# FerrisMind/candle-video

Measured on AMD Instinct MI355X. Metric: frames/sec end-to-end LTX-Video-2B 512x768x97; DiT step ms; VAE decode ms, higher is better.
Workload: dtype bf16; 1 GPU; LTX-Video-0.9.8-2B-distilled 512x768x97, 7 steps (configs.rs:223-240), untiled VAE decode; preset=0.9.8-2b-distilled, denoise_steps=7, parallelism=replicas x1 (no data-path collective)

## Files before the change

### candle-video_amd/csrc/capi_ops.hip

```cpp
#include "model_util.h"
#include "../../include/ltxhip_ops.h"

static inline int dtc(int d) { return d == 1 ? LTX_DT_BF16 : LTX_DT_F32; }

extern "C" int ltx_op_linear(const void* x, const void* w, const void* bias, void* y, int M, int N, int K, int dtype, int epi,
                             const void* resid, const float* gate, int rows_per_batch, ltx_stream stream) {
    if (!x || !w || !y) LTX_FAIL(LTX_ERR_ARG, "ltx_op_linear: null tensor");
    if (epi < 0 || epi > 3) LTX_FAIL(LTX_ERR_ARG, "ltx_op_linear: epi must be 0..3");
    if ((epi == 2 || epi == 3) && !resid) LTX_FAIL(LTX_ERR_ARG, "ltx_op_linear: residual epilogue needs resid");
    if (epi == 2 && (!gate || rows_per_batch < 1)) LTX_FAIL(LTX_ERR_ARG, "ltx_op_linear: gated epilogue needs gate");
    GemmArgs g; g.A = x; g.W = w; g.C = y; g.bias = bias; g.resid = resid; g.gate = gate;
    g.M = M; g.N = N; g.K = K; g.lda = K; g.ldc = N; g.ldr = N; g.rows_per_batch = rows_per_batch > 0 ? rows_per_batch : 1; g.gate_stride = N;
    return ltx_launch_gemm(g, dtc(dtype), epi, (hipStream_t)stream);
}

extern "C" int64_t ltx_op_ring_packed_bytes(int N, int K) { return (int64_t)ltx_ring_packed_bytes(N, K); }
extern "C" int ltx_op_ring_pack(const void* w, int N, int K, void* out, ltx_stream stream) { return ltx_pack_ring_weights(w, N, K, out, (hipStream_t)stream); }
extern "C" int ltx_op_linear_packed(const void* x, const void* w, const void* w_packed, const void* bias, void* y, int M, int N, int K, int epi,
                                    const void* resid, const float* gate, int rows_per_batch, ltx_stream stream) {
    if (!x || !w || !w_packed || !y) LTX_FAIL(LTX_ERR_ARG, "ltx_op_linear_packed: null tensor");
    if (epi < 0 || epi > 3) LTX_FAIL(LTX_ERR_ARG, "ltx_op_linear_packed: epi must be 0..3");
    if ((epi == 2 || epi == 3) && !resid) LTX_FAIL(LTX_ERR_ARG, "ltx_op_linear_packed: residual epilogue needs resid");
    if (epi == 2 && (!gate || rows_per_batch < 1)) LTX_FAIL(LTX_ERR_ARG, "ltx_op_linear_packed: gated epilogue needs gate");
    GemmArgs g; g.A = x; g.W = w; g.Wp = w_packed; g.C = y; g.bias = bias; g.resid = resid; g.gate = gate;
// ... 135 lines not shown
    if (hipMemcpy(dtab, tab, sizeof(tab), hipMemcpyHostToDevice) != hipSuccess) rc = LTX_ERR_HIP;
    if (rc == LTX_OK) {
        TimeVec tv; tv.n = n;
        for (int i = 0; i < n; ++i) tv.t[i] = timesteps_host[i];
        rc = ltx_launch_sinusoid(out, dtc(dtype), tv, dtab, 128, dtc(dtype) == LTX_DT_BF16, multiplier, (hipStream_t)stream);
        if (rc == LTX_OK && hipStreamSynchronize((hipStream_t)stream) != hipSuccess) rc = LTX_ERR_HIP;
    }
    (void)hipFree(dtab);
    return rc;
}

extern "C" int ltx_op_qknorm_rope(void* x, int64_t rows, int D, int ld, const void* weight, float eps,
                                  const float* cos, const float* sin, int dtype, ltx_stream stream) {
    if (!x || !weight) LTX_FAIL(LTX_ERR_ARG, "ltx_op_qknorm_rope: null tensor");
    QkNormRopeArgs a; a.x = x; a.rows = rows; a.D = D; a.ld = ld; a.nseg = 1; a.w0 = weight; a.eps = eps; a.cos = cos; a.sin = sin;
    return ltx_launch_qknorm_rope(a, dtc(dtype), (hipStream_t)stream);
}

extern "C" int ltx_op_rope_table(float* cos, float* sin, const float* coords, int B, int F, int H, int W, int D,
                                 const float* rope_scale_host, ltx_stream stream) {
    if (!cos || !sin) LTX_FAIL(LTX_ERR_ARG, "ltx_op_rope_table: null tensor");
    int steps = D / 6; if (steps < 1) steps = 1;
    std::vector<float> fr(steps);
    const float theta_ln = (float)std::log(10000.0);
    for (int i = 0; i < steps; ++i) {
        float lin = steps <= 1 ? 0.0f : (float)i * (float)(1.0 / (double)(steps - 1));
        fr[i] = (float)std::exp((double)(lin * theta_ln)) * (float)(M_PI / 2.0);
    }
    float* dfr = nullptr;
    HIP_TRY(hipMalloc((void**)&dfr, sizeof(float) * steps));
// ... 166 lines not shown
```

### candle-video_amd/csrc/dit.hip

```cpp
#include <cstring>
#include <deque>
#include "model_util.h"
#include "options.h"
#include "../../include/ltxhip_cond.h"
#include "lora.h"

struct DitBlock {
    LinearW qkv1, o1, q2, kv2, o2, ff1, ff2;
    void *nq1 = nullptr, *nk1 = nullptr, *nq2 = nullptr, *nk2 = nullptr;
};

struct DitCtx {
    const void* enc = nullptr; const float* mask = nullptr;
    int B = 0, K = 0, iodt = 0; bool valid = false;
    bool fold_q2 = false;
    DevBuf kv, bias;
    bool compact = false;
    DevBuf kvc, biasc, kidx, kcount;
    void release() { kv.release(); bias.release(); kvc.release(); biasc.release(); kidx.release(); kcount.release(); valid = false; }
};

struct DitTimeEntry {
    float t[8] = {0}; int B = 0; hipStream_t stream = nullptr; bool valid = false; uint64_t used = 0;
    DevBuf ada, adaf;
// ... 18 lines not shown
    int device = 0;
    int D = 0;
    LinearW proj_in, te1, te2, te_lin, cap1, cap2, proj_out;
    void* sst_final = nullptr;
    void* sst_blocks = nullptr;
    std::vector<DitBlock> blocks;
    float* rope_freqs = nullptr;
    float* inv_freq = nullptr;
    std::vector<int> skip_blocks;
    std::deque<DitCtx> ctxs;
    bool ctx_mode = false;
    std::deque<DitTimeEntry> tcache; uint64_t tclock = 0;
    std::deque<DitWfold> wcache;
    std::deque<DitGroupEntry> gcache;
    bool wfold_off = false;
    struct { bool valid = false; const float* coords = nullptr; float rs[3] = {0, 0, 0}; bool has_rs = false; int B = 0, S = 0, F = 0, H = 0, W = 0; hipStream_t stream = nullptr; } rope_key;
    void invalidate_weight_derived() {
        for (auto& e : wcache) e.valid = false;
        for (auto& e : ctxs) e.valid = false;
        for (auto& e : tcache) e.cfold_valid = false;
        for (auto& e : gcache) e.cfold_valid = false;
    }
    void release_scaled_weights() { for (auto& e : wcache) e.release(); }
    void release_caches() { auto all = [](auto& c) { for (auto& e : c) e.release(); c.clear(); }; all(ctxs); all(tcache); all(wcache); all(gcache); }
    std::vector<void*> owned;
    struct LoraSlots { void* base[7] = {nullptr}; void* merged[7] = {nullptr}; };
    std::vector<LoraSlots> lora_w;
    int n_adapters = 0;
    DevBuf xin, encin, h, n, qkv, attn, ff, c1, encp, kv2, tproj, e1, emb, embs, temb, ada, adaf, cosb, sinb, bias, orig, orig_hsq, outT, rsq, hsq, parts;
    void free_all() {
        for (void* p : owned) if (p) (void)hipFree(p);
        owned.clear();
        for (auto& ls : lora_w) for (void*& p : ls.merged) if (p) { (void)hipFree(p); p = nullptr; }
        lora_w.clear();
        DevBuf* bs[] = {&xin, &encin, &h, &n, &qkv, &attn, &ff, &c1, &encp, &kv2, &tproj, &e1, &emb, &embs, &temb, &ada, &adaf, &cosb, &sinb, &bias, &orig, &orig_hsq, &outT, &rsq, &hsq, &parts};
        for (DevBuf* b : bs) b->release();
        release_caches();
    }
};

namespace {

int own_linear(ltx_dit* m, const WeightMap& wm, const std::string& prefix, int in, int out, LinearW* l) {
    LTX_TRY(ltx_load_linear(wm, prefix, in, out, m->dtype, l));
    m->owned.push_back(l->w); if (l->b) m->owned.push_back(l->b);
    return LTX_OK;
}
int own_tensor(ltx_dit* m, const WeightMap& wm, const std::string& name, int64_t numel, void** out) {
    LTX_TRY(ltx_load_tensor(wm, name, numel, m->dtype, out));
    m->owned.push_back(*out);
// ... 370 lines not shown
    RopeTableArgs r;
    r.cos = m->cosb.as<float>(); r.sin = m->sinb.as<float>(); r.freqs = m->rope_freqs;
    r.B = p.B; r.D = p.D;
    if (video_coords) {
        r.use_coords = 1; r.coords = video_coords; r.F = 1; r.H = 1; r.W = p.S;
        r.gscale[0] = (float)(1.0 / 20.0); r.gscale[1] = (float)(1.0 / 2048.0); r.gscale[2] = (float)(1.0 / 2048.0);
    } else {
        r.F = num_frames; r.H = height; r.W = width;
        if (rope_scale) {
            r.gscale[0] = (float)((double)rope_scale[0] * c.patch_size_t / 20.0);
            r.gscale[1] = (float)((double)rope_scale[1] * c.patch_size / 2048.0);
            r.gscale[2] = (float)((double)rope_scale[2] * c.patch_size / 2048.0);
        }
    }
    LTX_TRY(ltx_launch_rope_table(r, s));
    rk.coords = video_coords; rk.B = p.B; rk.S = p.S; rk.F = num_frames; rk.H = height; rk.W = width; rk.stream = s;
    rk.has_rs = rope_scale != nullptr; if (rope_scale) memcpy(rk.rs, rope_scale, sizeof(rk.rs));
    rk.valid = m->ctx_mode;
    return LTX_OK;
}

struct DitCarry {
    bool hsq_valid = false;
    bool hs_valid = false;
    bool hsq_saved = false;
    bool pending = false; const float* pend_gate = nullptr; const void* pend_bias = nullptr;
    void take_pending(RowNormArgs& rn, const ltx_dit* m, const DitPlan& p) {
        if (!pending) return;
        rn.parts = m->parts.as<float>(); rn.nparts = p.ff2_parts; rn.part_stride = p.M * p.D; rn.d_bias = pend_bias; rn.d_gate = pend_gate; rn.d_gate_stride = 6 * p.D;
        rn.x_out = m->h.p; pending = false;
// ... 31 lines not shown
                  ln >= 0 ? in.tab.ada + (size_t)ln * NB * 6 * D : nullptr, p.nfold ? in.tab.cfold + (size_t)l * NB * 7 * D : nullptr,
                  wf ? (const char*)in.we->w.p + (size_t)l * 7 * D * D * esz : nullptr, c.norm_eps};
    const DitForm fold_in_form = wf ? kFold2 : kFold1;
    RowNormArgs rn; rn.x = m->h.p; rn.y = m->n.p; rn.rows = M; rn.D = D; rn.ldx = D; rn.ldy = D;
    rn.kind = 0; rn.eps = c.norm_eps; rn.shift = ada; rn.scale = ada + D; rn.rows_per_batch = p.Sg; rn.mod_stride = 6 * D;
    if (p.presum && st.hsq_valid) { rn.presum = m->hsq.as<float>(); rn.presum_n = D / 128; }
    const bool fold1 = p.nfold && st.hsq_valid && (wf || st.hs_valid);
    if (!fold1) { st.take_pending(rn, m, p); LTX_TRY(ltx_launch_rownorm(rn, dt, s)); }
    st.hs_valid = false;
    rn.parts = nullptr; rn.nparts = 0; rn.x_out = nullptr; rn.d_bias = nullptr; rn.d_gate = nullptr;
    LTX_TRY(ltx_launch_gemm(gemm_qkv1(p, fold1 ? fold_in_form : kPass, b, x), dt, EPI_BIAS, s));
    const float attn_scale = 1.0f / std::sqrt((float)hd);
    QkNormRopeArgs qa; qa.x = m->qkv.p; qa.rows = M; qa.D = D; qa.ld = p.ldqkv; qa.seg_stride = p.seg; qa.nseg = 2; qa.w0 = b.nq1; qa.w1 = b.nk1;
    qa.eps = 1e-5f; qa.cos = m->cosb.as<float>(); qa.sin = m->sinb.as<float>();
    if (p.fold_q) qa.out_scale0 = attn_scale * 1.4426950408889634f;
    LTX_TRY(ltx_launch_qknorm_rope(qa, dt, s));
    AttnArgs at; at.q = m->qkv.p; at.k = (char*)m->qkv.p + (size_t)p.seg * esz; at.v = (char*)m->qkv.p + (size_t)2 * p.seg * esz; at.o = m->attn.p;
    at.ldq = at.ldk = at.ldv = p.ldqkv; at.ldo = D; at.B = B; at.Sq = S; at.Sk = S; at.heads = H; at.hd = hd; at.scale = attn_scale;
    at.q_prescaled = p.fold_q ? 1 : 0;
    LTX_TRY(ltx_launch_attention(at, dt, s));
    LTX_TRY(ltx_linear(b.o1, m->attn.p, D, m->h.p, D, (int)M, dt, EPI_GATE_RESID, s, m->h.p, D, ada + 2 * D, 6 * D, p.Sg));
    st.hsq_valid = false;
    const DitCtx* ctx = in.ctx;
    const char* kvl = (const char*)(ctx->compact ? ctx->kvc.p : ctx->kv.p) + (size_t)l * p.MK * 2 * D * esz;
    AttnArgs ax; ax.q = m->qkv.p; ax.k = kvl; ax.v = kvl + (size_t)D * esz; ax.o = m->attn.p;
    ax.ldq = D; ax.ldk = ax.ldv = 2 * D; ax.ldo = D; ax.B = B; ax.Sq = S; ax.Sk = p.K; ax.heads = H; ax.hd = hd; ax.scale = attn_scale;
    ax.bias = ctx->mask ? ctx->bias.as<float>() : nullptr;
    if (ctx->compact) { ax.bias = ctx->biasc.as<float>(); ax.k_count = ctx->kcount.as<int>(); }
    if (p.fold_q2) {
        LTX_TRY(ltx_launch_gemm(gemm_q2(p, b, x), dt, EPI_BIAS, s));
// ... 45 lines not shown
    if (!video_coords && (int64_t)num_frames * height * width != S)
        LTX_FAIL(LTX_ERR_ARG, "ltx_dit_forward: num_frames*height*width must equal S when video_coords is absent");
    HIP_TRY(hipSetDevice(m->device));
    if (G < 1 || S % G != 0) LTX_FAIL(LTX_ERR_ARG, "ltx_dit_forward: the modulation groups must divide the sequence");
    hipStream_t s = (hipStream_t)stream;
    const ltx_dit_config& c = m->cfg;
    const DitPlan p = ltx_dit_plan(c, m->dtype, io_dtype == LTX_BF16 ? LTX_DT_BF16 : LTX_DT_F32, B, S, K, G, skip_layer_mask != nullptr);
    const int dt = p.dt, D = p.D, L = c.num_layers;
    const int64_t M = p.M, MK = p.MK; const size_t esz = ltx_dt_size(dt);
    const size_t nte = p.NB == p.B ? (size_t)p.B : 8;
    const size_t MD = M * D * esz, KD = MK * D * esz, part = M * (D / 128) * sizeof(float), rope = M * (D / 2) * sizeof(float);
    const std::pair<DevBuf*, size_t> ws[] = {
        {&m->xin, M * c.in_channels * esz}, {&m->encin, MK * c.caption_channels * esz}, {&m->h, MD}, {&m->n, MD}, {&m->qkv, 3 * MD}, {&m->attn, MD}, {&m->ff, 4 * MD},
        {&m->c1, KD}, {&m->encp, KD}, {&m->kv2, 2 * KD}, {&m->tproj, nte * 256 * esz}, {&m->e1, nte * D * esz}, {&m->emb, nte * D * esz}, {&m->embs, nte * D * esz},
        {&m->temb, nte * 6 * D * esz}, {&m->cosb, rope}, {&m->sinb, rope}, {&m->bias, MK * sizeof(float)}, {&m->outT, M * c.out_channels * esz},
        {&m->rsq, p.fold_q2 ? part : 0}, {&m->hsq, p.presum ? part : 0}, {&m->parts, p.defer_ff2 ? (size_t)p.ff2_parts * M * D * sizeof(float) : 0}, {&m->orig, skip_layer_mask ? MD : 0}};
    for (const auto& w : ws) LTX_TRY(w.first->ensure(w.second));

    LTX_TRY(ltx_launch_cast(hidden, p.iodt, m->xin.p, dt, p.M * c.in_channels, s));
    LTX_TRY(ltx_linear(m->proj_in, m->xin.p, c.in_channels, m->h.p, D, (int)p.M, dt, EPI_BIAS, s));

    DitLayerIn in; in.skip_layer_mask = skip_layer_mask;
    LTX_TRY(G == 1 ? time_tables(m, p, timestep, B, s, &in.tab) : group_tables(m, p, timestep, s, &in.tab));
    LTX_TRY(scaled_weights(m, p, timestep, in.tab.ada, s, &in.we));
    DitCtx* ctx = nullptr;
    LTX_TRY(text_context(m, p, enc, enc_mask, s, &ctx)); in.ctx = ctx;
    LTX_TRY(rope_tables(m, p, num_frames, height, width, rope_scale, video_coords, s));

    DitCarry st;
    for (int l = 0; l < L; ++l)
        if (block_runs(m, skip_layer_mask, B, l)) LTX_TRY(dit_block(m, p, l, in, st, s));
// ... 160 lines not shown
```

### candle-video_amd/csrc/kernels.h

```cpp
#pragma once
#include <hip/hip_runtime.h>
#include <hip/hip_ext.h>
#include <stdint.h>

enum { LTX_DT_F32 = 0, LTX_DT_BF16 = 1 };
static inline size_t ltx_dt_size(int dt) { return dt == LTX_DT_BF16 ? 2 : 4; }

enum { LTX_PROF_GEMM = 0, LTX_PROF_CONV = 1, LTX_PROF_ATTN_SELF = 2, LTX_PROF_ATTN_CROSS = 3, LTX_PROF_ROWNORM = 4, LTX_PROF_NKINDS = 5 };
bool ltx_prof_begin(int kind, double work, hipStream_t s, void** token);
void ltx_prof_end(void* token, hipStream_t s);
enum { LTX_PROFK_GEMM128 = 0, LTX_PROFK_GEMM_BIG = 1, LTX_PROFK_GEMM_P8 = 2, LTX_PROFK_CONV_HALO = 3, LTX_PROFK_GEMM_ASM = 4, LTX_PROFK_GEMM_ASM16 = 5, LTX_PROFK_GEMM_RING = 6, LTX_PROFK_N = 7 };
void ltx_prof_kernel(int which);
bool ltx_prof_kernel_events(hipEvent_t* a, hipEvent_t* b);
#define LTX_LAUNCH_TIMED(kernel, grid, block, shmem, stream, ...) do {                                           \
        hipEvent_t _pa = nullptr, _pb = nullptr;                                                                   \
        if (ltx_prof_kernel_events(&_pa, &_pb)) hipExtLaunchKernelGGL(kernel, grid, block, shmem, stream, _pa, _pb, 0, __VA_ARGS__); \
        else hipLaunchKernelGGL(kernel, grid, block, shmem, stream, __VA_ARGS__);                                  \
    } while (0)

enum { EPI_BIAS = 0, EPI_GELU = 1, EPI_GATE_RESID = 2, EPI_RESID = 3, EPI_D2S = 4, EPI_UNPATCH = 5, EPI_S2D = 6 };

struct GemmArgs {
    const void* A = nullptr;
    const void* W = nullptr;
// ... 80 lines not shown
    const float* presum = nullptr; int presum_n = 0;
    const float* parts = nullptr; int nparts = 0; int64_t part_stride = 0;
    const void* d_bias = nullptr; const float* d_gate = nullptr; int d_gate_stride = 0; void* x_out = nullptr;
};
int ltx_launch_rownorm(const RowNormArgs& a, int dtype, hipStream_t s);

struct QkNormRopeArgs {
    void* x = nullptr;
    int64_t rows = 0; int D = 0; int ld = 0; int nseg = 1;
    int64_t seg_stride = 0;
    const void* w0 = nullptr; const void* w1 = nullptr;
    const void* w0b = nullptr;
    float eps = 1e-5f;
    const float* cos = nullptr; const float* sin = nullptr;
    float out_scale0 = 1.f;
};
int ltx_launch_qknorm_rope(const QkNormRopeArgs& a, int dtype, hipStream_t s);

struct RopeTableArgs {
    float* cos = nullptr; float* sin = nullptr;
    const float* coords = nullptr;
    const float* freqs = nullptr;
    int B = 1, F = 1, H = 1, W = 1, D = 0;
    int use_coords = 0;
    float gscale[3] = {1.f, 1.f, 1.f};
};
int ltx_launch_rope_table(const RopeTableArgs& a, hipStream_t s);

struct AttnArgs {
    const void* q = nullptr; const void* k = nullptr; const void* v = nullptr; void* o = nullptr;
    int ldq = 0, ldk = 0, ldv = 0, ldo = 0;
// ... 77 lines not shown
```

### candle-video_amd/csrc/options.cpp

```cpp
#include "options.h"
#include <atomic>
#include <cstdio>
#include <cstdlib>
#include <cstring>
#include <map>
#include <mutex>
#include <string>
#include "errors.h"

namespace {
std::mutex g_mu;
LtxOptions g_opt;
std::atomic<bool> g_loaded{false};
std::map<std::string, int> g_exp;

struct ListBit { const char* name; unsigned bit; };
const ListBit kFam[] = {{"asm16", LTX_FAM_ASM16}, {"ring", LTX_FAM_RING}, {"p8", LTX_FAM_P8}, {"halo", LTX_FAM_HALO}, {"halo_out", LTX_FAM_HALO_OUT}, {"big", LTX_FAM_BIG}};
const ListBit kAttn[] = {{"q64", LTX_ATTN_Q64}, {"q128", LTX_ATTN_Q128}, {"cross", LTX_ATTN_CROSS}, {"pipe", LTX_ATTN_PIPE}};

template <size_t N> bool parse_list(const char* v, const ListBit (&tab)[N], unsigned* out) {
    unsigned bits = 0;
    std::string s(v ? v : "");
    size_t p = 0;
    while (p < s.size()) {
        size_t q = s.find('+', p); if (q == std::string::npos) q = s.size();
        const std::string item = s.substr(p, q - p);
        bool ok = item.empty();
        for (const auto& t : tab) if (item == t.name) { bits |= t.bit; ok = true; }
        if (!ok) return false;
        p = q + 1;
    }
    *out = bits;
    return true;
}

struct IntField { const char* name; int LtxOptions::*field; };
const IntField kInts[] = {
    {"gemm_tune", &LtxOptions::gemm_tune}, {"gemm_wide_epi", &LtxOptions::gemm_wide_epi}, {"gemm_trace", &LtxOptions::gemm_trace},
    {"attn_q64_big", &LtxOptions::attn_q64_big}, {"vae_tile_batch", &LtxOptions::vae_tile_batch}, {"prof_kernel_events", &LtxOptions::prof_kernel_events}, {"ff2_defer", &LtxOptions::ff2_defer},
    {"gemm_splitk", &LtxOptions::gemm_splitk}, {"q2_fold", &LtxOptions::q2_fold}, {"norm_presum", &LtxOptions::norm_presum}, {"norm_lean", &LtxOptions::norm_lean},
    {"xattn_compact", &LtxOptions::xattn_compact}, {"dense_qkv", &LtxOptions::dense_qkv}, {"vae_fuse_norm", &LtxOptions::vae_fuse_norm}, {"t5_attn_mfma", &LtxOptions::t5_attn_mfma}, {"guidance_batch", &LtxOptions::guidance_batch}, {"norm_fold", &LtxOptions::norm_fold}, {"norm_fold_copies", &LtxOptions::norm_fold_copies}, {"attn_q64_stream", &LtxOptions::attn_q64_stream},
};

bool set_one(LtxOptions& o, const std::string& key, const char* value) {
    static const LtxOptions dflt;
    for (const auto& f : kInts) if (key == f.name) {
        if (!value) { o.*(f.field) = dflt.*(f.field); return true; }
        char* end = nullptr; const long v = strtol(value, &end, 10);
        if (end == value || *end) return false;
        o.*(f.field) = (int)v; return true;
    }
    if (key == "gemm_plan") {
        if (!value) { o.gemm_plan[0] = 0; return true; }
        if (strlen(value) >= sizeof(o.gemm_plan)) return false;
// ... 88 lines not shown
```

### candle-video_amd/csrc/options.h

```cpp
#pragma once

enum { LTX_FAM_ASM16 = 1, LTX_FAM_RING = 2, LTX_FAM_P8 = 4, LTX_FAM_HALO = 8, LTX_FAM_HALO_OUT = 16, LTX_FAM_BIG = 32 };
enum { LTX_ATTN_Q64 = 1, LTX_ATTN_Q128 = 2, LTX_ATTN_CROSS = 4, LTX_ATTN_PIPE = 8 };

struct LtxOptions {
    int gemm_tune = 1;
    char gemm_plan[40] = {0};
    unsigned gemm_off = 0;
    int gemm_wide_epi = 1;
    int gemm_trace = 0;
    int attn_q64_big = -1;
    int vae_tile_batch = 0;
    int prof_kernel_events = 1;
    int ff2_defer = 1;
    int gemm_splitk = 1;
    int q2_fold = 1;
    int norm_presum = 1;
    int norm_lean = 1;
    int xattn_compact = 1;
    int attn_q64_stream = 0;
    int norm_fold = 2;
    int norm_fold_copies = 10;
    int guidance_batch = 1;
    int dense_qkv = 1;
    int vae_fuse_norm = 1;
    int t5_attn_mfma = 1;
    unsigned attn_off = 0;
};

// ... 8 lines not shown
```

### candle-video_amd/csrc/rownorm.hip

```cpp
#include <type_traits>
#include "common.h"
#include "kernels.h"
#include "gemm_common.h"
#include "options.h"

namespace {

constexpr int NSLOT = 8;

__device__ __forceinline__ float group_sum(float v, int lpr) {
    for (int o = lpr >> 1; o > 0; o >>= 1) v += __shfl_xor(v, o);
    return v;
}

template <typename T>
__device__ __forceinline__ void finish_chunk(const RowNormArgs& a, const float* f_in, float mean, float rinv, int c, const float* sc,
                                             const float* sh, T* y, bool active) {
    constexpr int CH = ElemTraits<T>::CHUNK;
    const T* w = reinterpret_cast<const T*>(a.weight);
    float f[CH], wv[CH], scv[CH], shv[CH];
    if (w) { Chunk16 wc; wc.u = *reinterpret_cast<const u32x4*>(w + c * CH); chunk_to_f32<T>(wc, wv); }
    if (sc) {
#pragma unroll
        for (int q = 0; q < CH / 4; ++q) {
// ... 517 lines not shown
        } else {
            float ss = 0.f;
            for (int c = sub; c < nch; c += lpr) {
                Chunk16 v; v.u = *reinterpret_cast<const u32x4*>(x + c * CH);
                float f[CH]; chunk_to_f32<T>(v, f);
#pragma unroll
                for (int i = 0; i < CH; ++i) ss += f[i] * f[i];
            }
            ss = group_sum(ss, lpr);
            const float rinv = oscale / sqrtf(ss / (float)a.D + a.eps);
            for (int c = sub; c < nch; c += lpr) { Chunk16 v; v.u = *reinterpret_cast<const u32x4*>(x + c * CH); finish(v, c, rinv, w, wb, x); }
        }
    }
}

template <typename T, int NS, int OCC = 5>
__global__ __launch_bounds__(256, OCC) void qknorm_rope_fused_kernel(const QkNormRopeArgs a, int lpr) {
    constexpr int CH = ElemTraits<T>::CHUNK;
    static_assert(CH == 8, "bf16 rows only");
    const int lane = threadIdx.x & 63, wave = threadIdx.x >> 6;
    const int rpw = 64 / lpr;
    const int64_t row = ((int64_t)blockIdx.x * 4 + wave) * rpw + lane / lpr;
    const int sub = lane % lpr;
    const bool active = row < a.rows;
    const int64_t rr = active ? row : a.rows - 1;
    const int nch = a.D / CH;
    const bool rope = a.cos != nullptr;
    const float* cs = rope ? a.cos + rr * (a.D / 2) : nullptr;
    const float* sn = rope ? a.sin + rr * (a.D / 2) : nullptr;
    T* x0 = reinterpret_cast<T*>(a.x) + rr * a.ld;
    const int64_t sst = a.seg_stride ? a.seg_stride : a.D;
    Chunk16 v[2][NS];
    f32x4 co[NS], si[NS];
#pragma unroll
    for (int i = 0; i < NS; ++i) {
        const int c = sub + i * lpr;
        const bool in = c < nch;
        v[0][i].u = (u32x4){0u, 0u, 0u, 0u}; v[1][i].u = (u32x4){0u, 0u, 0u, 0u};
        if (in) v[0][i].u = *reinterpret_cast<const u32x4*>(x0 + c * CH);
        if (in && a.nseg == 2) v[1][i].u = *reinterpret_cast<const u32x4*>(x0 + sst + c * CH);
        if (in && rope) { co[i] = *reinterpret_cast<const f32x4*>(cs + c * 4); si[i] = *reinterpret_cast<const f32x4*>(sn + c * 4); }
    }
    float rinv[2] = {0.f, 0.f};
#pragma unroll
    for (int seg = 0; seg < 2; ++seg) {
        if (seg >= a.nseg) break;
        float ss = 0.f;
#pragma unroll
        for (int i = 0; i < NS; ++i) { float f[CH]; chunk_to_f32<T>(v[seg][i], f);
#pragma unroll
            for (int j = 0; j < CH; ++j) ss += f[j] * f[j]; }
        ss = group_sum(ss, lpr);
        rinv[seg] = (seg == 0 ? a.out_scale0 : 1.0f) / sqrtf(ss / (float)a.D + a.eps);
    }
#pragma unroll
    for (int i = 0; i < NS; ++i) {
// ... 305 lines not shown
            *reinterpret_cast<u32x4*>(x0 + seg * sst + c * CH) = o.u;
        }
    }
}
}

int ltx_launch_qknorm_rope(const QkNormRopeArgs& a, int dtype, hipStream_t s) {
    const int ch = dtype == LTX_DT_BF16 ? 8 : 4;
    if (a.rows <= 0) return LTX_OK;
    if (a.D % ch != 0 || a.ld % ch != 0) LTX_FAIL(LTX_ERR_ARG, "qknorm: D/ld must be multiples of the 16-byte chunk");
    if (a.nseg < 1 || a.nseg > 2 || !a.w0 || (a.nseg == 2 && !a.w1)) LTX_FAIL(LTX_ERR_ARG, "qknorm: bad segments/weights");
    const int nch = a.D / ch, lpr = pick_lpr(nch);
    const int64_t rows_per_block = 4 * (64 / lpr);
    dim3 grid((unsigned)cdiv64(a.rows, rows_per_block)), block(256);
    const bool cached = nch <= NSLOT * lpr;
    if (dtype == LTX_DT_BF16) {
        if (a.rows <= 512 && nch > 64 && nch <= 512) hipLaunchKernelGGL((qknorm_rope_block_kernel<bf16_t>), dim3((unsigned)a.rows), block, 0, s, a);
        else if (nch <= 4 * lpr) hipLaunchKernelGGL((qknorm_rope_fused_kernel<bf16_t, 4>), grid, block, 0, s, a, lpr);
        else if (nch <= 8 * lpr && ltx_exp("qknorm_fused8", 1)) hipLaunchKernelGGL((qknorm_rope_fused_kernel<bf16_t, 8, 2>), grid, block, 0, s, a, lpr);
        else if (cached) hipLaunchKernelGGL((qknorm_rope_kernel<bf16_t, true>), grid, block, 0, s, a, lpr);
        else hipLaunchKernelGGL((qknorm_rope_kernel<bf16_t, false>), grid, block, 0, s, a, lpr);
    } else {
        if (cached) hipLaunchKernelGGL((qknorm_rope_kernel<float, true>), grid, block, 0, s, a, lpr);
        else hipLaunchKernelGGL((qknorm_rope_kernel<float, false>), grid, block, 0, s, a, lpr);
    }
    LTX_CHECK_LAUNCH();
    return LTX_OK;
}

int ltx_launch_rowsq(const void* x, int dtype, int64_t rows, int N, int ld, float* out, hipStream_t s) {
    if (rows <= 0 || N <= 0) return LTX_OK;
    if (!x || !out || N % 4 != 0 || ld % 4 != 0 || ((uintptr_t)x & 7)) LTX_FAIL(LTX_ERR_ARG, "rowsq: N and ld must be multiples of 4 and x 8-byte aligned");
    const int64_t npairs = rows * ((N + 127) / 128);
// ... 43 lines not shown
        LTX_FAIL(LTX_ERR_ARG, "shift_gemv: bf16 weights [N, K] with K % 8 == 0, f32 shift rows 16-byte aligned, 1..8 batch rows");
    hipLaunchKernelGGL(shift_gemv_kernel, dim3((unsigned)((N + 3) / 4)), dim3(256), 0, s, reinterpret_cast<const bf16_t*>(W), reinterpret_cast<const bf16_t*>(bias),
                       shift, shift_stride, B, N, K, cvec, cvec_stride);
    LTX_CHECK_LAUNCH();
    return LTX_OK;
}

int ltx_launch_rope_table(const RopeTableArgs& a, hipStream_t s) {
    if (a.D % 2 != 0 || a.D < 6) LTX_FAIL(LTX_ERR_ARG, "rope: dim must be even and >= 6");
    const int64_t total = (int64_t)a.B * a.F * a.H * a.W * (a.D / 2);
    int64_t blocks = cdiv64(total, 256); if (blocks > 8192) blocks = 8192;
    hipLaunchKernelGGL(rope_table_kernel, dim3((unsigned)blocks), dim3(256), 0, s, a);
    LTX_CHECK_LAUNCH();
    return LTX_OK;
}
```

### candle-video_amd/ltxhip/__init__.py

```python
from __future__ import annotations

import ctypes as C
import os
from dataclasses import dataclass, field
from typing import Dict, List, Optional, Sequence, Tuple

import torch

_HERE = os.path.dirname(os.path.abspath(__file__))
_LIB_PATH = os.environ.get("LTXHIP_LIB") or os.path.join(os.path.dirname(_HERE), "libltxhip.so")

if not os.path.exists(_LIB_PATH):
    raise ImportError(
        f"ltxhip: {_LIB_PATH} is missing — build it with `make -C candle-video_amd` "
        "(or `python -c 'import __graft_entry__ as g; g.build()'`). There is no CPU fallback.")
lib = C.CDLL(_LIB_PATH)

LTX_F32, LTX_BF16 = 0, 1


class LtxError(RuntimeError):
    pass


# ... 81 lines not shown
    "ltx_op_ring_packed_bytes": [_i, _i], "ltx_op_ring_pack": [_vp, _i, _i, _vp, _vp],
    "ltx_op_linear_packed": [_vp, _vp, _vp, _vp, _vp, _i, _i, _i, _i, _vp, _vp, _i, _vp],
    "ltx_op_rownorm_presum": [_vp, _vp, _i64, _i, _f, _vp, _vp, _vp, _i64, _i, _i, _vp, _i, _i, _vp],
    "ltx_op_linear_rowsq": [_vp, _vp, _vp, _vp, _vp, _i, _i, _i, _i, _i, _vp, _vp, _i, _vp], "ltx_op_rowsq": [_vp, _i64, _i, _i, _vp, _i, _vp],
    "ltx_op_linear_fold_out": [_vp, _vp, _vp, _vp, _vp, _vp, _vp, _i, _i, _i, _i, _i, _vp, _vp, _i, _vp],
    "ltx_op_linear_fold_in": [_vp, _vp, _vp, _vp, _i, _i, _f, _vp, _i, _i, _i, _i, _i, _i, _vp],
    "ltx_op_linear_fold_ok": [_i, _i, _i, _i, _i, _i, _i, _i],
    "ltx_op_shift_gemv": [_vp, _vp, _vp, _i, _i, _i, _i, _vp, _i, _vp],
    "ltx_op_mod_scale": [_vp, _vp, _i, _vp, _i, _i64, _i, _i, _vp], "ltx_op_scale_cols": [_vp, _vp, _vp, _i64, _i, _i, _vp],
    "ltx_op_linear_split_factor": [_i, _i, _i], "ltx_op_linear_deferred": [_vp, _vp, _vp, _i, _i, _i, _vp],
    "ltx_op_rownorm_deferred": [_vp, _i, _vp, _vp, _vp, _i, _vp, _vp, _i64, _i, _i, _f, _vp, _vp, _i64, _i, _i, _vp],
    "ltx_op_attention_compact": [_vp, _vp, _vp, _vp, _i, _i, _i, _i, _i, _i, _i, _i, _i, _f, _vp, _vp, _i, _i, _f, _vp, _vp],
    "ltx_op_attention_rowsq": [_vp, _vp, _vp, _vp, _i, _i, _i, _i, _i, _i, _i, _i, _i, _f, _vp, _vp, _i, _i, _f, _vp],
    "ltx_op_rownorm": [_vp, _vp, _i64, _i, _i, _f, _vp, _vp, _vp, _i64, _i, _i, _i, _vp],
    "ltx_op_qknorm_rope": [_vp, _i64, _i, _i, _vp, _f, _vp, _vp, _i, _vp],
    "ltx_op_rope_table": [_vp, _vp, _vp, _i, _i, _i, _i, _i, _vp, _vp],
    "ltx_op_timestep_embedding": [_vp, _i, _i, _f, _i, _vp, _vp],
    "ltx_op_attention": [_vp, _vp, _vp, _vp, _i, _i, _i, _i, _i, _i, _i, _i, _i, _f, _vp, _i, _vp],
    "ltx_op_attention_prescaled": [_vp, _vp, _vp, _vp, _i, _i, _i, _i, _i, _i, _i, _i, _i, _vp],
    "ltx_op_conv3d": [_vp, _vp, _vp, _i, _vp, _vp, _i, _i, _i, _i, _i, _i, _i, _i, _vp],
    "ltx_op_upsample3d": [_vp, _vp, _vp, _i, _vp, _i, _i, _i, _i, _i, _i, _i, _i, _i, _vp],
    "ltx_op_conv_out_unpatchify": [_vp, _vp, _vp, _i, _vp, _i, _i, _i, _i, _i, _i, _i, _i, _i, _vp],
    "ltx_op_blend": [_vp, _vp, _i, _i, _i, _i, _i, _i, _i, _i, _i, _vp],
    "ltx_op_downsample3d": [_vp, _vp, _vp, _i, _vp, _i, _i, _i, _i, _i, _i, _i, _i, _vp],
    "ltx_op_gemm_plan": [_i, _i, _i, _i, _i, _i, _i, _i, C.c_char_p, _i],
    "ltx_op_gemm_route": [_i, _i, _i, _i, _i, _i, _i, _i, _i, _i, _i, _i, C.c_char_p, _i],
    "ltx_op_dit_plan": [_i, _i, _i, _i, _i, _i, _i, _i, _i, C.POINTER(C.c_int64)],
    "ltx_t5_config_default": [_vp], "ltx_t5_create": [_vp, _vp, _sz, _i, _i, _vp], "ltx_t5_destroy": [_vp],
    "ltx_t5_forward": [_vp, _vp, _i, _i, _i, _vp, _vp],
    "ltx_t5_create_from_gguf": [_vp, C.c_char_p, _i, _i, _vp], "ltx_t5_forward_masked": [_vp, _vp, _vp, _i, _i, _i, _vp, _vp],
# ... 1364 lines not shown
        y = torch.empty_like(x)
        ms = scale.shape[-1] if scale is not None else 0
        _check(lib.ltx_op_rownorm_presum(_ptr(x.contiguous()), _ptr(y), C.c_int64(rows), D, C.c_float(eps), _ptr(weight), _ptr(scale), _ptr(shift),
                                         C.c_int64(rows_per_batch), ms, act, _ptr(presum), presum.shape[-1], _dt(x.dtype), _stream()))
        return y

    @staticmethod
    def qknorm_rope(x, weight, eps=1e-5, cos=None, sin=None):
        x = x.clone().contiguous()
        rows, D = x.shape
        _check(lib.ltx_op_qknorm_rope(_ptr(x), C.c_int64(rows), D, D, _ptr(weight), C.c_float(eps), _ptr(cos), _ptr(sin),
                                      _dt(x.dtype), _stream()))
        return x

    @staticmethod
    def timestep_embedding(timesteps, vae_flavour=False, multiplier=1.0, dtype=torch.float32, device="cuda"):
        ts = [float(t) for t in timesteps]
        out = torch.empty(len(ts), 256, dtype=dtype, device=device)
        _check(lib.ltx_op_timestep_embedding(_floats(ts), len(ts), int(bool(vae_flavour)), C.c_float(multiplier), _dt(dtype), _ptr(out), _stream()))
        return out

    @staticmethod
    def rope_table(B, F, H, W, D, coords=None, rope_scale=None, device="cuda"):
        cos = torch.empty(B * F * H * W, D // 2, dtype=torch.float32, device=device)
        sin = torch.empty_like(cos)
        _check(lib.ltx_op_rope_table(_ptr(cos), _ptr(sin), _ptr(coords), B, F, H, W, D,
                                     _floats(rope_scale) if rope_scale is not None else None, _stream()))
        return cos, sin

    @staticmethod
# ... 104 lines not shown
```

### include/ltxhip_ops.h

```cpp
#ifndef LTXHIP_OPS_H
#define LTXHIP_OPS_H
#include "ltxhip.h"
#ifdef __cplusplus
extern "C" {
#endif

int ltx_op_linear(const void* x, const void* w, const void* bias, void* y, int M, int N, int K, int dtype, int epi,
                  const void* resid, const float* gate, int rows_per_batch, ltx_stream stream);

int64_t ltx_op_ring_packed_bytes(int N, int K);
int ltx_op_ring_pack(const void* w, int N, int K, void* out, ltx_stream stream);
int ltx_op_linear_packed(const void* x, const void* w, const void* w_packed, const void* bias, void* y, int M, int N, int K, int epi,
                         const void* resid, const float* gate, int rows_per_batch, ltx_stream stream);
int ltx_op_linear_rowsq(const void* x, const void* w, const void* bias, void* y, float* rowsq, int M, int N, int K, int dtype, int epi,
                        const void* resid, const float* gate, int rows_per_batch, ltx_stream stream);
int ltx_op_rowsq(const void* x, int64_t rows, int N, int ld, float* rowsq, int dtype, ltx_stream stream);

int ltx_op_linear_fold_out(const void* x, const void* w, const void* bias, void* y, void* y2, float* rowsq, const float* scale2, int scale2_stride,
                           int M, int N, int K, int epi, const void* resid, const float* gate, int rows_per_batch, ltx_stream stream);
int ltx_op_linear_fold_in(const void* x, const void* w, void* y, const float* rs_sq, int rs_n, int rs_D, float eps, const float* cvec, int cvec_stride,
                          int M, int N, int K, int epi, int rows_per_batch, ltx_stream stream);
int ltx_op_linear_fold_ok(int M, int N, int K, int epi, int consumer, int rs_n, int vec_stride, int rows_per_batch);
int ltx_op_shift_gemv(const void* w, const void* bias, const float* shift, int shift_stride, int B, int N, int K, float* cvec, int cvec_stride, ltx_stream stream);
int ltx_op_mod_scale(const void* h, const float* scale, int scale_stride, void* y, int B, int64_t rows_per_batch, int D, int dtype, ltx_stream stream);
// ... 7 lines not shown
                          const float* presum, int presum_n, int dtype, ltx_stream stream);

int ltx_op_linear_split_factor(int M, int N, int K);
int ltx_op_linear_deferred(const void* x, const void* w, float* parts, int M, int N, int K, ltx_stream stream);
int ltx_op_rownorm_deferred(const float* parts, int nparts, const void* bias, const void* resid, const float* gate, int gate_stride, void* h_out,
                            void* y, int64_t rows, int D, int kind, float eps, const float* scale, const float* shift, int64_t rows_per_batch,
                            int mod_stride, int dtype, ltx_stream stream);

int ltx_op_rownorm(const void* x, void* y, int64_t rows, int D, int kind, float eps, const void* weight,
                   const float* scale, const float* shift, int64_t rows_per_batch, int mod_stride, int act,
                   int dtype, ltx_stream stream);

int ltx_op_qknorm_rope(void* x, int64_t rows, int D, int ld, const void* weight, float eps,
                       const float* cos, const float* sin, int dtype, ltx_stream stream);

int ltx_op_timestep_embedding(const float* timesteps_host, int n, int vae_flavour, float multiplier, int dtype, void* out, ltx_stream stream);

int ltx_op_rope_table(float* cos, float* sin, const float* coords, int B, int F, int H, int W, int D,
                      const float* rope_scale_host, ltx_stream stream);

int ltx_op_attention(const void* q, const void* k, const void* v, void* o, int B, int Sq, int Sk, int heads, int hd,
                     int ldq, int ldk, int ldv, int ldo, float scale, const float* key_bias, int dtype, ltx_stream stream);
int ltx_attention_fallback_counts(unsigned long long counts[2], int reset);
int ltx_op_attention_rowsq(const void* q, const void* k, const void* v, void* o, int B, int Sq, int Sk, int heads, int hd,
                           int ldq, int ldk, int ldv, int ldo, float scale, const float* key_bias,
                           const float* q_rowsq, int q_rowsq_n, int q_rowsq_D, float q_rowsq_eps, ltx_stream stream);
int ltx_op_attention_compact(const void* q, const void* k, const void* v, void* o, int B, int Sq, int Sk, int heads, int hd,
                             int ldq, int ldk, int ldv, int ldo, float scale, const float* key_bias,
                             const float* q_rowsq, int q_rowsq_n, int q_rowsq_D, float q_rowsq_eps, int* counts_out, ltx_stream stream);
int ltx_op_attention_prescaled(const void* q, const void* k, const void* v, void* o, int B, int Sq, int Sk, int heads, int hd,
// ... 32 lines not shown
```

Baseline: 538.5 frames/sec.

## Exploit separable RoPE tables in fused qk-norm kernel to cut table reads

Adds a device-side check for whether video RoPE coordinates split into a frame part and a spatial part. When they do, the fused qk-norm+RoPE kernel reads cos/sin from two small, highly cached row subsets (frame row and spatial row) and merges them per element by a mod-3 pattern, instead of streaming a full per-token table. The check runs once per rope-table build, and a device flag lets the kernel fall back to per-row offsets if the check fails. This adds extra address arithmetic and explicit scheduling barriers in a memory-bound kernel, plus a test API.

Result: no change. 540.3 frames/sec (median of 6 runs) (+0.3%).

```diff
diff --git a/candle-video_amd/csrc/capi_ops.hip b/candle-video_amd/csrc/capi_ops.hip
--- a/candle-video_amd/csrc/capi_ops.hip
+++ b/candle-video_amd/csrc/capi_ops.hip
@@ -173,6 +173,14 @@
                                   const float* cos, const float* sin, int dtype, ltx_stream stream) {
     if (!x || !weight) LTX_FAIL(LTX_ERR_ARG, "ltx_op_qknorm_rope: null tensor");
     QkNormRopeArgs a; a.x = x; a.rows = rows; a.D = D; a.ld = ld; a.nseg = 1; a.w0 = weight; a.eps = eps; a.cos = cos; a.sin = sin;
+    return ltx_launch_qknorm_rope(a, dtc(dtype), (hipStream_t)stream);
+}
+
+extern "C" int ltx_op_qknorm_rope_qk(void* x, int64_t rows, int D, int ld, int64_t seg_stride, const void* wq, const void* wk, float eps,
+                                     const float* cos, const float* sin, float out_scale0, int S, int HW, int shared, int dtype, ltx_stream stream) {
+    if (!x || !wq || !wk) LTX_FAIL(LTX_ERR_ARG, "ltx_op_qknorm_rope_qk: null tensor");
+    QkNormRopeArgs a; a.x = x; a.rows = rows; a.D = D; a.ld = ld; a.seg_stride = seg_stride; a.nseg = 2; a.w0 = wq; a.w1 = wk; a.eps = eps; a.cos = cos; a.sin = sin;
+    a.out_scale0 = out_scale0; a.rope_shared = shared ? 1 : 0; a.S = S; a.HW = HW;
     return ltx_launch_qknorm_rope(a, dtc(dtype), (hipStream_t)stream);
 }
 
diff --git a/candle-video_amd/csrc/dit.hip b/candle-video_amd/csrc/dit.hip
--- a/candle-video_amd/csrc/dit.hip
+++ b/candle-video_amd/csrc/dit.hip
@@ -56,7 +56,8 @@
     std::deque<DitWfold> wcache;
     std::deque<DitGroupEntry> gcache;
     bool wfold_off = false;
-    struct { bool valid = false; const float* coords = nullptr; float rs[3] = {0, 0, 0}; bool has_rs = false; int B = 0, S = 0, F = 0, H = 0, W = 0; hipStream_t stream = nullptr; } rope_key;
+    struct { bool valid = false; const float* coords = nullptr; float rs[3] = {0, 0, 0}; bool has_rs = false; int B = 0, S = 0, F = 0, H = 0, W = 0; hipStream_t stream = nullptr;
+             int sep = 0; } rope_key;
     void invalidate_weight_derived() {
         for (auto& e : wcache) e.valid = false;
         for (auto& e : ctxs) e.valid = false;
@@ -69,13 +70,13 @@
     struct LoraSlots { void* base[7] = {nullptr}; void* merged[7] = {nullptr}; };
     std::vector<LoraSlots> lora_w;
     int n_adapters = 0;
-    DevBuf xin, encin, h, n, qkv, attn, ff, c1, encp, kv2, tproj, e1, emb, embs, temb, ada, adaf, cosb, sinb, bias, orig, orig_hsq, outT, rsq, hsq, parts;
+    DevBuf xin, encin, h, n, qkv, attn, ff, c1, encp, kv2, tproj, e1, emb, embs, temb, ada, adaf, cosb, sinb, bias, orig, orig_hsq, outT, rsq, hsq, parts, ropeflag;
     void free_all() {
         for (void* p : owned) if (p) (void)hipFree(p);
         owned.clear();
         for (auto& ls : lora_w) for (void*& p : ls.merged) if (p) { (void)hipFree(p); p = nullptr; }
         lora_w.clear();
-        DevBuf* bs[] = {&xin, &encin, &h, &n, &qkv, &attn, &ff, &c1, &encp, &kv2, &tproj, &e1, &emb, &embs, &temb, &ada, &adaf, &cosb, &sinb, &bias, &orig, &orig_hsq, &outT, &rsq, &hsq, &parts};
+        DevBuf* bs[] = {&xin, &encin, &h, &n, &qkv, &attn, &ff, &c1, &encp, &kv2, &tproj, &e1, &emb, &embs, &temb, &ada, &adaf, &cosb, &sinb, &bias, &orig, &orig_hsq, &outT, &rsq, &hsq, &parts, &ropeflag};
         for (DevBuf* b : bs) b->release();
         release_caches();
     }
@@ -476,6 +477,12 @@
         }
     }
     LTX_TRY(ltx_launch_rope_table(r, s));
+    rk.sep = 0;
+    if (!video_coords) rk.sep = 1;
+    else if (num_frames >= 1 && height >= 1 && width >= 1 && (int64_t)num_frames * height * width == p.S) {
+        LTX_TRY(ltx_launch_rope_separable(video_coords, p.B, p.S, height * width, m->ropeflag.as<int>(), s));
+        rk.sep = 2;
+    }
     rk.coords = video_coords; rk.B = p.B; rk.S = p.S; rk.F = num_frames; rk.H = height; rk.W = width; rk.stream = s;
     rk.has_rs = rope_scale != nullptr; if (rope_scale) memcpy(rk.rs, rope_scale, sizeof(rk.rs));
     rk.valid = m->ctx_mode;
@@ -537,6 +544,10 @@
     QkNormRopeArgs qa; qa.x = m->qkv.p; qa.rows = M; qa.D = D; qa.ld = p.ldqkv; qa.seg_stride = p.seg; qa.nseg = 2; qa.w0 = b.nq1; qa.w1 = b.nk1;
     qa.eps = 1e-5f; qa.cos = m->cosb.as<float>(); qa.sin = m->sinb.as<float>();
     if (p.fold_q) qa.out_scale0 = attn_scale * 1.4426950408889634f;
+    if (m->rope_key.sep && ltx_opt().rope_shared) {
+        qa.rope_shared = 1; qa.S = S; qa.HW = m->rope_key.H * m->rope_key.W;
+        if (m->rope_key.sep == 2) qa.shared_flag = m->ropeflag.as<int>();
+    }
     LTX_TRY(ltx_launch_qknorm_rope(qa, dt, s));
     AttnArgs at; at.q = m->qkv.p; at.k = (char*)m->qkv.p + (size_t)p.seg * esz; at.v = (char*)m->qkv.p + (size_t)2 * p.seg * esz; at.o = m->attn.p;
     at.ldq = at.ldk = at.ldv = p.ldqkv; at.ldo = D; at.B = B; at.Sq = S; at.Sk = S; at.heads = H; at.hd = hd; at.scale = attn_scale;
@@ -612,7 +623,7 @@
         {&m->xin, M * c.in_channels * esz}, {&m->encin, MK * c.caption_channels * esz}, {&m->h, MD}, {&m->n, MD}, {&m->qkv, 3 * MD}, {&m->attn, MD}, {&m->ff, 4 * MD},
         {&m->c1, KD}, {&m->encp, KD}, {&m->kv2, 2 * KD}, {&m->tproj, nte * 256 * esz}, {&m->e1, nte * D * esz}, {&m->emb, nte * D * esz}, {&m->embs, nte * D * esz},
         {&m->temb, nte * 6 * D * esz}, {&m->cosb, rope}, {&m->sinb, rope}, {&m->bias, MK * sizeof(float)}, {&m->outT, M * c.out_channels * esz},
-        {&m->rsq, p.fold_q2 ? part : 0}, {&m->hsq, p.presum ? part : 0}, {&m->parts, p.defer_ff2 ? (size_t)p.ff2_parts * M * D * sizeof(float) : 0}, {&m->orig, skip_layer_mask ? MD : 0}};
+        {&m->rsq, p.fold_q2 ? part : 0}, {&m->hsq, p.presum ? part : 0}, {&m->parts, p.defer_ff2 ? (size_t)p.ff2_parts * M * D * sizeof(float) : 0}, {&m->orig, skip_layer_mask ? MD : 0}, {&m->ropeflag, sizeof(int)}};
     for (const auto& w : ws) LTX_TRY(w.first->ensure(w.second));
 
     LTX_TRY(ltx_launch_cast(hidden, p.iodt, m->xin.p, dt, p.M * c.in_channels, s));
diff --git a/candle-video_amd/csrc/kernels.h b/candle-video_amd/csrc/kernels.h
--- a/candle-video_amd/csrc/kernels.h
+++ b/candle-video_amd/csrc/kernels.h
@@ -118,7 +118,9 @@
     float eps = 1e-5f;
     const float* cos = nullptr; const float* sin = nullptr;
     float out_scale0 = 1.f;
-};
+    int rope_shared = 0; int S = 0, HW = 0; const int* shared_flag = nullptr;
+};
+int ltx_launch_rope_separable(const float* coords, int B, int S, int HW, int* flag, hipStream_t s);
 int ltx_launch_qknorm_rope(const QkNormRopeArgs& a, int dtype, hipStream_t s);
 
 struct RopeTableArgs {
diff --git a/candle-video_amd/csrc/options.cpp b/candle-video_amd/csrc/options.cpp
--- a/candle-video_amd/csrc/options.cpp
+++ b/candle-video_amd/csrc/options.cpp
@@ -37,7 +37,7 @@
 struct IntField { const char* name; int LtxOptions::*field; };
 const IntField kInts[] = {
     {"gemm_tune", &LtxOptions::gemm_tune}, {"gemm_wide_epi", &LtxOptions::gemm_wide_epi}, {"gemm_trace", &LtxOptions::gemm_trace},
-    {"attn_q64_big", &LtxOptions::attn_q64_big}, {"vae_tile_batch", &LtxOptions::vae_tile_batch}, {"prof_kernel_events", &LtxOptions::prof_kernel_events}, {"ff2_defer", &LtxOptions::ff2_defer},
+    {"attn_q64_big", &LtxOptions::attn_q64_big}, {"vae_tile_batch", &LtxOptions::vae_tile_batch}, {"prof_kernel_events", &LtxOptions::prof_kernel_events}, {"ff2_defer", &LtxOptions::ff2_defer}, {"rope_shared", &LtxOptions::rope_shared},
     {"gemm_splitk", &LtxOptions::gemm_splitk}, {"q2_fold", &LtxOptions::q2_fold}, {"norm_presum", &LtxOptions::norm_presum}, {"norm_lean", &LtxOptions::norm_lean},
     {"xattn_compact", &LtxOptions::xattn_compact}, {"dense_qkv", &LtxOptions::dense_qkv}, {"vae_fuse_norm", &LtxOptions::vae_fuse_norm}, {"t5_attn_mfma", &LtxOptions::t5_attn_mfma}, {"guidance_batch", &LtxOptions::guidance_batch}, {"norm_fold", &LtxOptions::norm_fold}, {"norm_fold_copies", &LtxOptions::norm_fold_copies}, {"attn_q64_stream", &LtxOptions::attn_q64_stream},
 };
diff --git a/candle-video_amd/csrc/options.h b/candle-video_amd/csrc/options.h
--- a/candle-video_amd/csrc/options.h
+++ b/candle-video_amd/csrc/options.h
@@ -13,6 +13,7 @@
     int vae_tile_batch = 0;
     int prof_kernel_events = 1;
     int ff2_defer = 1;
+    int rope_shared = 1;
     int gemm_splitk = 1;
     int q2_fold = 1;
     int norm_presum = 1;
diff --git a/candle-video_amd/csrc/rownorm.hip b/candle-video_amd/csrc/rownorm.hip
--- a/candle-video_amd/csrc/rownorm.hip
+++ b/candle-video_amd/csrc/rownorm.hip
@@ -555,7 +555,7 @@
     }
 }
 
-template <typename T, int NS, int OCC = 5>
+template <typename T, int NS, int OCC = 5, bool SH = false>
 __global__ __launch_bounds__(256, OCC) void qknorm_rope_fused_kernel(const QkNormRopeArgs a, int lpr) {
     constexpr int CH = ElemTraits<T>::CHUNK;
     static_assert(CH == 8, "bf16 rows only");
@@ -569,18 +569,66 @@
     const bool rope = a.cos != nullptr;
     const float* cs = rope ? a.cos + rr * (a.D / 2) : nullptr;
     const float* sn = rope ? a.sin + rr * (a.D / 2) : nullptr;
+    unsigned offp = 0, offf = 0;
+    if constexpr (SH) {
+        const bool on = !a.shared_flag || *a.shared_flag != 0;
+        const unsigned r = (unsigned)rr, sl = r % (unsigned)a.S, fhw = sl / (unsigned)a.HW * (unsigned)a.HW;
+        offp = (on ? r - fhw : r) * (unsigned)(a.D * 2); offf = (on ? r - sl + fhw : r) * (unsigned)(a.D * 2);
+    }
+    const unsigned rem3 = 3u - (unsigned)(a.D % 6) / 2u;
     T* x0 = reinterpret_cast<T*>(a.x) + rr * a.ld;
     const int64_t sst = a.seg_stride ? a.seg_stride : a.D;
     Chunk16 v[2][NS];
     f32x4 co[NS], si[NS];
+    constexpr int NU = 2 * NS, NH = NU / 2;
+    f32x4 tp[NH], tf[NH];
+    auto issue = [&](int u) {
+        const int c = sub + (u >> 1) * lpr, cc = c < nch ? c : 0;
+        const char* tab = reinterpret_cast<const char*>((u & 1) ? a.sin : a.cos);
+        tp[u % NH] = *reinterpret_cast<const f32x4*>(tab + (offp + (unsigned)cc * 16u)); tf[u % NH] = *reinterpret_cast<const f32x4*>(tab + (offf + (unsigned)cc * 16u));
+    };
+    auto merge = [&](int u) {
+        const unsigned m = ((unsigned)(sub + (u >> 1) * lpr) + rem3) % 3u;
+        const bool f0 = m == 0, f1 = m == 2, f2 = m == 1;
+        const f32x4 p = tp[u % NH], f = tf[u % NH];
+        f32x4 t = (f32x4){f0 ? f[0] : p[0], f1 ? f[1] : p[1], f2 ? f[2] : p[2], f0 ? f[3] : p[3]};
+        asm volatile("" : "+v"(t));
+        if (u & 1) si[u >> 1] = t; else co[u >> 1] = t;
+    };
+    if constexpr (SH) {
+#pragma unroll
+        for (int u = 0; u < NH; ++u) issue(u);
+        __builtin_amdgcn_sched_barrier(0);
+    }
 #pragma unroll
     for (int i = 0; i < NS; ++i) {
         const int c = sub + i * lpr;
         const bool in = c < nch;
+        if constexpr (SH) {
+            const int cc = in ? c : 0;
+            v[0][i].u = *reinterpret_cast<const u32x4*>(x0 + cc * CH); v[1][i].u = *reinterpret_cast<const u32x4*>(x0 + (a.nseg == 2 ? sst : 0) + cc * CH);
+            continue;
+        }
         v[0][i].u = (u32x4){0u, 0u, 0u, 0u}; v[1][i].u = (u32x4){0u, 0u, 0u, 0u};
         if (in) v[0][i].u = *reinterpret_cast<const u32x4*>(x0 + c * CH);
         if (in && a.nseg == 2) v[1][i].u = *reinterpret_cast<const u32x4*>(x0 + sst + c * CH);
-        if (in && rope) { co[i] = *reinterpret_cast<const f32x4*>(cs + c * 4); si[i] = *reinterpret_cast<const f32x4*>(sn + c * 4); }
+        if constexpr (!SH) {
+            if (in && rope) { co[i] = *reinterpret_cast<const f32x4*>(cs + c * 4); si[i] = *reinterpret_cast<const f32x4*>(sn + c * 4); }
+        }
+    }
+    if constexpr (SH) {
+        __builtin_amdgcn_sched_barrier(0);
+#pragma unroll
+        for (int u = 0; u < NH; ++u) merge(u);
+        __builtin_amdgcn_sched_barrier(0);
+#pragma unroll
+        for (int u = NH; u < NU; ++u) issue(u);
+        __builtin_amdgcn_sched_barrier(0);
+#pragma unroll
+        for (int u = NH; u < NU; ++u) merge(u);
+        __builtin_amdgcn_sched_barrier(0);
+#pragma unroll
+        for (int i = 0; i < NS; ++i) if (sub + i * lpr >= nch) { v[0][i].u = (u32x4){0u, 0u, 0u, 0u}; v[1][i].u = (u32x4){0u, 0u, 0u, 0u}; }
     }
     float rinv[2] = {0.f, 0.f};
 #pragma unroll
@@ -916,9 +964,13 @@
     const int64_t rows_per_block = 4 * (64 / lpr);
     dim3 grid((unsigned)cdiv64(a.rows, rows_per_block)), block(256);
     const bool cached = nch <= NSLOT * lpr;
+    if (a.rope_shared && (a.S < 1 || a.HW < 1 || a.S % a.HW != 0 || a.rows % a.S != 0)) LTX_FAIL(LTX_ERR_ARG, "qknorm: shared table rows need rows = B * S and S = F * HW");
+    const bool sh = a.rope_shared && a.cos && a.sin && a.rows * a.D * 2 < ((int64_t)1 << 32);
     if (dtype == LTX_DT_BF16) {
         if (a.rows <= 512 && nch > 64 && nch <= 512) hipLaunchKernelGGL((qknorm_rope_block_kernel<bf16_t>), dim3((unsigned)a.rows), block, 0, s, a);
+        else if (nch <= 4 * lpr && sh) hipLaunchKernelGGL((qknorm_rope_fused_kernel<bf16_t, 4, 5, true>), grid, block, 0, s, a, lpr);
         else if (nch <= 4 * lpr) hipLaunchKernelGGL((qknorm_rope_fused_kernel<bf16_t, 4>), grid, block, 0, s, a, lpr);
+        else if (nch <= 8 * lpr && sh && ltx_exp("qknorm_fused8", 1)) hipLaunchKernelGGL((qknorm_rope_fused_kernel<bf16_t, 8, 2, true>), grid, block, 0, s, a, lpr);
         else if (nch <= 8 * lpr && ltx_exp("qknorm_fused8", 1)) hipLaunchKernelGGL((qknorm_rope_fused_kernel<bf16_t, 8, 2>), grid, block, 0, s, a, lpr);
         else if (cached) hipLaunchKernelGGL((qknorm_rope_kernel<bf16_t, true>), grid, block, 0, s, a, lpr);
         else hipLaunchKernelGGL((qknorm_rope_kernel<bf16_t, false>), grid, block, 0, s, a, lpr);
@@ -992,3 +1044,18 @@
     LTX_CHECK_LAUNCH();
     return LTX_OK;
 }
+
+static __global__ void rope_separable_kernel(const uint32_t* coords, int64_t rows, int S, int HW, int* flag) {
+    const int64_t r = (int64_t)blockIdx.x * blockDim.x + threadIdx.x;
+    if (r >= rows) return;
+    const int64_t sl = r % S, fhw = sl / HW * HW, rp = r - fhw, rf = r - sl + fhw;
+    if (coords[r * 3] != coords[rf * 3] || coords[r * 3 + 1] != coords[rp * 3 + 1] || coords[r * 3 + 2] != coords[rp * 3 + 2]) *flag = 0;
+}
+int ltx_launch_rope_separable(const float* coords, int B, int S, int HW, int* flag, hipStream_t s) {
+    if (!coords || !flag || B < 1 || S < 1 || HW < 1 || S % HW != 0) LTX_FAIL(LTX_ERR_ARG, "rope: separability check needs coords [B, S, 3] with S = F * HW");
+    HIP_TRY(hipMemsetD32Async((hipDeviceptr_t)flag, 1, 1, s));
+    const int64_t rows = (int64_t)B * S;
+    hipLaunchKernelGGL(rope_separable_kernel, dim3((unsigned)cdiv64(rows, 256)), dim3(256), 0, s, reinterpret_cast<const uint32_t*>(coords), rows, S, HW, flag);
+    LTX_CHECK_LAUNCH();
+    return LTX_OK;
+}
diff --git a/candle-video_amd/ltxhip/__init__.py b/candle-video_amd/ltxhip/__init__.py
--- a/candle-video_amd/ltxhip/__init__.py
+++ b/candle-video_amd/ltxhip/__init__.py
@@ -119,6 +119,7 @@
     "ltx_op_attention_rowsq": [_vp, _vp, _vp, _vp, _i, _i, _i, _i, _i, _i, _i, _i, _i, _f, _vp, _vp, _i, _i, _f, _vp],
     "ltx_op_rownorm": [_vp, _vp, _i64, _i, _i, _f, _vp, _vp, _vp, _i64, _i, _i, _i, _vp],
     "ltx_op_qknorm_rope": [_vp, _i64, _i, _i, _vp, _f, _vp, _vp, _i, _vp],
+    "ltx_op_qknorm_rope_qk": [_vp, _i64, _i, _i, _i64, _vp, _vp, _f, _vp, _vp, _f, _i, _i, _i, _i, _vp],
     "ltx_op_rope_table": [_vp, _vp, _vp, _i, _i, _i, _i, _i, _vp, _vp],
     "ltx_op_timestep_embedding": [_vp, _i, _i, _f, _i, _vp, _vp],
     "ltx_op_attention": [_vp, _vp, _vp, _vp, _i, _i, _i, _i, _i, _i, _i, _i, _i, _f, _vp, _i, _vp],
@@ -1513,6 +1514,15 @@
         return x
 
     @staticmethod
+    def qknorm_rope_qk(qk, wq, wk, cos, sin, eps=1e-5, out_scale0=1.0, S=0, HW=0, shared=False):
+        qk = qk.clone().contiguous()
+        rows, D2 = qk.shape
+        D = D2 // 2
+        _check(lib.ltx_op_qknorm_rope_qk(_ptr(qk), C.c_int64(rows), D, D2, C.c_int64(D), _ptr(wq), _ptr(wk), C.c_float(eps), _ptr(cos), _ptr(sin),
+                                         C.c_float(out_scale0), S, HW, int(bool(shared)), _dt(qk.dtype), _stream()))
+        return qk
+
+    @staticmethod
     def timestep_embedding(timesteps, vae_flavour=False, multiplier=1.0, dtype=torch.float32, device="cuda"):
         ts = [float(t) for t in timesteps]
         out = torch.empty(len(ts), 256, dtype=dtype, device=device)
diff --git a/include/ltxhip_ops.h b/include/ltxhip_ops.h
--- a/include/ltxhip_ops.h
+++ b/include/ltxhip_ops.h
@@ -45,6 +45,9 @@
 int ltx_op_qknorm_rope(void* x, int64_t rows, int D, int ld, const void* weight, float eps,
                        const float* cos, const float* sin, int dtype, ltx_stream stream);
 
+int ltx_op_qknorm_rope_qk(void* x, int64_t rows, int D, int ld, int64_t seg_stride, const void* wq, const void* wk, float eps,
+                          const float* cos, const float* sin, float out_scale0, int S, int HW, int shared, int dtype, ltx_stream stream);
+
 int ltx_op_timestep_embedding(const float* timesteps_host, int n, int vae_flavour, float multiplier, int dtype, void* out, ltx_stream stream);
 
 int ltx_op_rope_table(float* cos, float* sin, const float* coords, int B, int F, int H, int W, int D,
```
